# google-deepmind/dqn_zoo

Hardware: NVIDIA H100
Metric: learner_grad_steps_per_sec (higher is better)
Workload: dtype f32 (f64 sum tree)

## Files before the change

### dqn_zoo_b200/_lib.py

```python

import ctypes as C
import os

from dqn_zoo_b200 import _build

i32, i64, f32, f64, u64 = C.c_int32, C.c_int64, C.c_float, C.c_double, C.c_uint64
vp = C.c_void_p

DZ_FLAG_BAD_VALUE, DZ_FLAG_BAD_INDEX, DZ_FLAG_BAD_TARGET, DZ_FLAG_ROOT_ZERO, DZ_FLAG_NONFINITE_WEIGHT = 1, 2, 4, 8, 16
DZ_FLAG_FRAME_POOL_FULL = 32
AGENT_KINDS = {'dqn': 0, 'double_q': 1, 'prioritized': 2, 'c51': 3, 'qrdqn': 4, 'rainbow': 5, 'iqn': 6}
OPTIMIZERS = {'adam': 0, 'rmsprop': 1}


class ReplayView(C.Structure):
  _fields_ = [('d_obs', vp), ('d_action', vp), ('d_reward', vp), ('d_discount', vp), ('capacity', i64),
              ('obs_bytes', i64), ('obs_stride', i64), ('d_tree', vp), ('first_leaf', i64), ('d_live', vp),
              ('d_id_at', vp), ('d_ids', vp), ('d_flags', vp),
              ('d_frames', vp), ('frame_bytes', i64), ('frame_stride', i64), ('obs_channels', i64),
              ('frame_capacity', i64), ('d_planes', vp), ('d_refcount', vp), ('d_hashes', vp), ('d_table', vp),
              ('table_size', i64), ('d_free', vp), ('d_pool_counters', vp), ('d_add_staging', vp)]


class AddRecord(C.Structure):
# ... 82 lines not shown
    'dz_replay_gather': (i32, [C.POINTER(ReplayView), vp, i32, vp, vp, vp, vp, vp, vp]),
    'dz_replay_update_priorities': (i32, [C.POINTER(ReplayView), vp, vp, i32, f64, i64, vp]),
    'dz_learner_plan_query': (i32, [C.POINTER(LearnerConfig), C.POINTER(LearnerPlan)]),
    'dz_learner_tensor_info': (i32, [C.POINTER(LearnerConfig), i32, C.c_char_p, C.POINTER(i64), C.POINTER(i32),
                                     C.POINTER(i64)]),
    'dz_learner_create': (i32, [C.POINTER(LearnerConfig), C.POINTER(LearnerBuffers), C.POINTER(vp)]),
    'dz_learner_destroy': (None, [vp]),
    'dz_learner_update': (i32, [vp, C.POINTER(Batch), C.POINTER(UpdateOutputs), i32, vp]),
    'dz_learner_learn': (i32, [vp, C.POINTER(ReplayView), i32, C.POINTER(LearnIO), vp]),
    'dz_learner_generate_randomness': (i32, [vp, u64, vp, vp, vp]),
    'dz_learner_generate_randomness_async': (i32, [vp, u64, vp, vp, vp]),
    'dz_learner_q_values': (i32, [vp, vp, vp, vp, vp, vp]),
    'dz_learner_act_batch': (i32, [vp, vp, i32, vp, vp, vp, f32, vp, vp, vp]),
    'dz_learner_act_batch_stream_noise': (i32, [vp, vp, i32, vp, vp, f32, vp, vp, vp]),
    'dz_learner_noise_stride': (i32, [C.POINTER(LearnerConfig), C.POINTER(i64)]),
    'dz_learner_generate_stream_noise': (i32, [vp, u64, i32, vp, vp]),
    'dz_learner_sync_target': (i32, [vp, vp]),
    'dz_test_u8_to_unit': (i32, [vp, vp]),
    'dz_atari_preprocess': (i32, [vp, vp, i32, vp, vp, vp, vp, i32, vp, i32, vp]),
    'dz_atari_preprocess_band_rows': (i32, []),
    'dz_jax_uniform': (i32, [vp, vp, i32, vp, vp]),
    'dz_test_threefry2x32': (i32, [C.c_uint32, C.c_uint32, C.c_uint32, C.c_uint32, vp]),
    'dz_test_learner_buffer': (i32, [vp, C.c_char_p, vp, vp]),
    'dz_test_copy': (i32, [vp, vp, i64, vp]),
    'dz_test_learner_trace': (i32, [vp, C.c_char_p, vp]),
    'dz_test_learner_mma_path': (i32, [vp, C.c_char_p, C.POINTER(i32)]),
    'dz_debug_timeline': (i32, [vp]),
    'dz_test_tc_pgemm_work': (i64, [i32, i32, i32]),
    'dz_test_tc_pgemm': (i32, [vp, i32, i32, i32, vp, i32, i32, i32, i32, i32, vp, vp, i64, i64, i32, i64, vp, i32, vp]),
    'dz_test_umma_gemm': (i32, [vp, i32, vp, i32, i32, i32, i32, i32, vp, i32, i32, vp, i32, vp, vp, vp, vp]),
    'dz_test_umma_gemm_path': (i32, [vp, i32, vp, i32, i32, i32, i32, i32, vp, i32, i32, vp, i32, vp, vp, vp, i32, vp]),
    'dz_test_fc_forward': (i32, [i32, i32, i32, i32, i32, i32, vp, vp, vp, vp, vp, i64, vp, vp, vp, i32, vp, C.POINTER(i32),
                                 C.POINTER(i64), vp]),
    'dz_test_conv1_forward': (i32, [i32, i32, i32, i32, vp, vp, vp, i64, vp, i32, vp, vp, vp]),
}

EXPORTS = tuple(_SIGNATURES)


def library_path():
  return _build.LIB_PATH


def _load():
  path = library_path()
  if not os.path.exists(path):
    raise ImportError('dqn_zoo_b200: %s is missing — run `python -c "import __graft_entry__ as g; g.build()"` '
                      '(there is no CPU fallback)' % path)
  lib = C.CDLL(path)
  for name, (res, args) in _SIGNATURES.items():
    fn = getattr(lib, name)
    fn.restype, fn.argtypes = res, args
  return lib


lib = _load()


def check(status):
  if status != 0:
    raise _ERRORS.get(status, DzError)(lib.dz_last_error().decode())


def call(name, *args):
  check(getattr(lib, name)(*args))
```

### dqn_zoo_b200/csrc/dz_learner.cu

```cuda
#include <algorithm>
#include <cmath>
#include <map>
#include <vector>

#include "dz_async.cuh"
#include "dz_gemm.cuh"
#include "dz_tc.cuh"
#include "dz_internal.cuh"
#include "dz_umma_net.cuh"

namespace dz {


struct TensorInfo {
  std::string name;
  int64_t shape[4];
  int ndim;
  int64_t offset, count;
};

struct Dims {
  int H, W, C;
  int h1, w1, h2, w2, h3, w3;
  int feat;
// ... 1085 lines not shown
  dz_learner_config cfg;
  dz_learner_buffers buf;
  Layout lay;
  ParamOffsets po;
  Dims d;
  int B;
  int n_head[3];
  float *act1[3], *act2[3], *act3[3];
  float *h1[3][2], *out[3], *outv[3];
  float *cosf[3], *hi[3], *E0;
  float* nn_partial;
  float* conv_partial;
  float* nt_partial;
  float *dout, *doutv, *dh1[2], *dact3, *dtmp[2], *dcol, *dact2, *dact1, *dhi;
  float* tn_partial[4];
  float *loss_terms, *scalars;
  unsigned int* ticket;
  const uint8_t** rows_sample[2];
  uint8_t* recon = nullptr;
  int64_t recon_bytes = 0;
  const uint8_t** rows_act;
  int32_t* s_a; float *s_r, *s_d, *s_w;
  float* q_scratch;
  int fc_splits, head_splits, conv_splits, nt_splits;
  bool pk_on;
  struct PkImg { float* hi; float* lo; int rows_pad, red_pad; };
  PkImg pk_act[3], pk_wT[2], pk_w, pk_actT, pk_dh1T, pk_dh1, pk_cos[3], pk_weT[2], pk_dET, pk_cosT;
  bool pk_embed_bwd;
  int pk_embed_wgrad_splits;
  float *pk_fwd_partial, *pk_wgrad_partial;
  int pk_fwd_splits, pk_wgrad_splits;
  SideStream side;
  SideStream side2;
  float* norm_parts;
  UmNet* um;
  char* um_ws;
  int um_npass;
  bool opt_smem_set = false;
};

namespace {

constexpr int kNormBlocks = kNumSMs * 4;

int pick_splits(int64_t tiles, int nkb, int max_splits) {
  int best = 1;
  int64_t best_cost = -1;
  for (int s = 1; s <= max_splits; ++s) {
    int64_t cost = ceil_div(tiles * s, kNumSMs) * (ceil_div(nkb, s) + 6);
    if (best_cost < 0 || cost < best_cost) { best_cost = cost; best = s; }
  }
  return best;
}

UmNetDesc make_um_desc(const dz_learner* l);

int64_t carve(dz_learner* l, char* base) {
  const dz_learner_config& c = l->cfg;
  const Dims& d = l->d;
  const int B = c.batch;
  Bump w{base};
  const bool rb = c.kind == DZ_RAINBOW, iqn = c.kind == DZ_IQN;
  int nh[3] = {1, 1, 1};
  if (iqn) { nh[0] = c.tau_samples_s_tm1; nh[1] = c.tau_samples_policy; nh[2] = c.tau_samples_s_t; }
  for (int p = 0; p < 3; ++p) l->n_head[p] = nh[p];
  for (int p = 0; p < 3; ++p) {
// ... 551 lines not shown
  f.nsrc = nsrc; f.splits = probs[0].splits; f.stride = probs[0].split_stride; f.M = probs[0].M; f.K = probs[0].K;
  f.dual = dual ? 1 : 0; f.mask = mask; f.out = out; f.out_hi = out_hi; f.out_lo = out_lo;
  for (int q = 0; q < nsrc; ++q) { f.partial[q] = probs[q].C; f.a_scale[q] = probs[q].a_scale; }
  return f;
}
int finish_nt_batch(const FinishNT* jobs, int njobs, void* stream) {
  FinishNTBatch fb;
  memset(&fb, 0, sizeof(fb));
  long long total = 0;
  for (int j = 0; j < njobs; ++j) { fb.f[j] = jobs[j]; total = std::max(total, (long long)jobs[j].M * jobs[j].K); }
  dim3 grid((unsigned)std::min<long long>(ceil_div(total, 256), kNumSMs * 8), (unsigned)njobs);
  DZ_LAUNCH(finish_nt_kernel, grid, 256, 0, stream, fb);
  return DZ_OK;
}
int finish_nt(const GemmProblem* probs, int nsrc, const float* mask, float* out, bool dual, void* stream) {
  FinishNT f = make_finish_nt(probs, nsrc, mask, out, dual);
  return finish_nt_batch(&f, 1, stream);
}

bool split_norm_active(const dz_learner* l);

int backward_torso(dz_learner* l, const uint8_t* const* rows0, void* stream) {
  const Dims& d = l->d;
  const ParamOffsets& o = l->po;
  const int B = l->B;
  float* G = l->buf.d_grads;
  const float* P = l->buf.d_online;
  FinishTNBatch fb;
  fb.n = 0;
  GemmBatch gb;
  if (l->um && l->cfg.kind == DZ_IQN) DZ_TRY(um_split_dact3(l->um, stream));
  float* norm_parts = split_norm_active(l) ? l->norm_parts : nullptr;
  if (l->um) {
    void* ws = l->side.fork(stream, stream);
    DZ_TRY(um_wgrad_conv3(l->um, ws));
    DZ_TRY(um_wgrad_finish_layer(l->um, 3, G + o.conv_w[2], G + o.conv_b[2], norm_parts, ws));
  } else {
    GemmProblem p = zero_problem();
    set_conv(p, A_CONV_F32, l->act2[0], B, d.h2, d.w2, 64, 3, 3, 1);
    p.B = l->dact3; p.N = 64; p.ldb = 64; p.ldc = 64;
    p.Cb = G + o.conv_b[2];
    int splits = (int)std::min<int64_t>(32, ceil_div(p.M, 64));
    p.splits = splits; p.split_stride = (long long)(p.K + 1) * 64; p.C = l->tn_partial[2];
    gb.n = 1; gb.p[0] = p;
    DZ_TRY(run_tn("conv3_wgrad", gb, l->side.fork(stream, stream)));
    fb.f[fb.n++] = FinishTN{p.C, splits, p.split_stride, p.K, 64, G + o.conv_w[2], nullptr, p.Cb, nullptr, nullptr, nullptr};
  }
  if (l->um) {
    DZ_TRY(um_backward_conv3(l->um, stream));
  } else {
    GemmProblem p = zero_problem();
    p.A = l->dact3; p.lda = 64; p.M = B * d.h3 * d.w3; p.N = 64; p.K = 576;
    p.B = P + o.conv_w[2]; p.ldb = 64; p.C = l->dcol; p.ldc = 576;
    gb.n = 1; gb.p[0] = p;
    DZ_TRY(run_nt("conv3_dgrad", gb, false, stream));
    long long total = (long long)B * d.h2 * d.w2 * 64;
    DZ_LAUNCH(col2im_kernel, (unsigned)ceil_div(total, 256), 256, 0, stream, l->dcol, l->act2[0], l->dact2, B, d.h2, d.w2, 64, 3, 3, 1,
              d.h3, d.w3);
  }
  if (l->um) {
    void* ws = l->side2.fork(stream, stream);
    DZ_TRY(um_wgrad_conv2(l->um, ws));
    DZ_TRY(um_wgrad_finish_layer(l->um, 2, G + o.conv_w[1], G + o.conv_b[1], norm_parts, ws));
  } else {
    GemmProblem p = zero_problem();
    set_conv(p, A_CONV_F32, l->act1[0], B, d.h1, d.w1, 32, 4, 4, 2);
    p.B = l->dact2; p.N = 64; p.ldb = 64; p.ldc = 64;
    p.Cb = G + o.conv_b[1];
    int splits = (int)std::min<int64_t>(32, ceil_div(p.M, 64));
    p.splits = splits; p.split_stride = (long long)(p.K + 1) * 64; p.C = l->tn_partial[1];
    gb.n = 1; gb.p[0] = p;
    DZ_TRY(run_tn("conv2_wgrad", gb, l->side.fork(stream, stream)));
    fb.f[fb.n++] = FinishTN{p.C, splits, p.split_stride, p.K, 64, G + o.conv_w[1], nullptr, p.Cb, nullptr, nullptr, nullptr};
  }
  if (l->um) {
    DZ_TRY(um_backward_conv2(l->um, stream));
  } else {
    GemmProblem p = zero_problem();
    p.A = l->dact2; p.lda = 64; p.M = B * d.h2 * d.w2; p.N = 64; p.K = 512;
    p.B = P + o.conv_w[1]; p.ldb = 64; p.C = l->dcol; p.ldc = 512;
    gb.n = 1; gb.p[0] = p;
    DZ_TRY(run_nt("conv2_dgrad", gb, false, stream));
    long long total = (long long)B * d.h1 * d.w1 * 32;
    DZ_LAUNCH(col2im_kernel, (unsigned)ceil_div(total, 256), 256, 0, stream, l->dcol, l->act1[0], l->dact1, B, d.h1, d.w1, 32, 4, 4, 2,
              d.h2, d.w2);
  }
  if (l->um) {
    void* ws = l->side.fork(stream, stream);
    DZ_TRY(um_wgrad_conv1(l->um, rows0, ws));
    DZ_TRY(um_wgrad_finish_layer(l->um, 1, G + o.conv_w[0], G + o.conv_b[0], norm_parts, ws));
    DZ_TRY(l->side2.join(stream));
    return l->side.join(stream);
  } else {
    GemmProblem p = zero_problem();
    set_conv(p, A_CONV_U8, rows0, B, d.H, d.W, d.C, 8, 8, 4);
    p.B = l->dact1; p.N = 32; p.ldb = 32; p.ldc = 32;
    p.Cb = G + o.conv_b[0];
    int splits = (int)std::min<int64_t>(64, ceil_div(p.M, 64));
    p.splits = splits; p.split_stride = (long long)(p.K + 1) * 32; p.C = l->tn_partial[0];
    gb.n = 1; gb.p[0] = p;
    DZ_TRY(run_tn("conv1_wgrad", gb, l->side.fork(stream, stream)));
    fb.f[fb.n++] = FinishTN{p.C, splits, p.split_stride, p.K, 32, G + o.conv_w[0], nullptr, p.Cb, nullptr, nullptr, nullptr};
  }
  void* ws = l->side.tail(stream);
  dim3 grid((unsigned)ceil_div(577 * 64, 256), fb.n);
  DZ_LAUNCH(finish_tn_kernel, grid, 256, 0, ws, fb);
  return l->side.join(stream);
}

int backward_plain(dz_learner* l, void* stream) {
  const Dims& d = l->d;
  const ParamOffsets& o = l->po;
  const int B = l->B;
  float* G = l->buf.d_grads;
  const float* P = l->buf.d_online;
  const bool shared = l->cfg.kind == DZ_DOUBLE_Q || l->cfg.kind == DZ_PRIORITIZED;
  GemmBatch gb;
  gb.n = 1;
  {
    GemmProblem p = zero_problem();
    p.a_mode = A_PLAIN; p.A = l->h1[0][0]; p.lda = 512; p.M = B; p.K = 512;
    p.B = l->dout; p.N = d.out; p.ldb = d.out; p.ldc = d.out;
    p.C = G + o.w2[0]; p.Cb = shared ? l->scalars + 8 + kNormBlocks : G + o.b2[0];
// ... 322 lines not shown
    DZ_TRY(forward_heads_plain(l, passes, np, B, stream, um));
  }

  LossArgs L;
  memset(&L, 0, sizeof(L));
  L.kind = c.kind; L.B = B; L.A = c.num_actions; L.atoms = c.num_atoms;
  L.out0 = l->out[0]; L.out1 = l->out[1]; L.out2 = l->out[2];
  L.adv0 = l->out[0]; L.val0 = l->outv[0]; L.adv1 = l->out[1]; L.val1 = l->outv[1]; L.adv2 = l->out[2]; L.val2 = l->outv[2];
  L.a = batch->d_a_tm1; L.r = batch->d_r_t; L.disc = batch->d_discount_t; L.w = batch->d_weights; L.taus0 = batch->d_taus;
  L.vmax = c.vmax; L.bound = c.grad_error_bound; L.kappa = c.huber_param;
  L.dout = l->dout; L.dadv = l->dout; L.dval = l->doutv;
  L.per_example = out->d_per_example; L.loss_terms = l->loss_terms;
  L.priorities = (c.kind == DZ_RAINBOW || c.kind == DZ_PRIORITIZED) ? out->d_priorities : nullptr;
  if (c.kind == DZ_DQN || c.kind == DZ_DOUBLE_Q || c.kind == DZ_PRIORITIZED) {
    DZ_LAUNCH(loss_q_kernel, B, 64, 0, stream, L);
  } else if (c.kind == DZ_C51 || c.kind == DZ_RAINBOW) {
    DZ_LAUNCH_NAMED("loss_categorical_kernel", loss_categorical_staged_kernel, B, 128, categorical_loss_smem(c), stream, L);
  } else {
    if (c.kind == DZ_QRDQN) { L.N = c.num_quantiles; L.Ksel = c.num_quantiles; L.Nt = c.num_quantiles; }
    else { L.N = c.tau_samples_s_tm1; L.Ksel = c.tau_samples_policy; L.Nt = c.tau_samples_s_t; }
    size_t smem = (32 + c.num_actions + L.Nt + 2 * L.N) * sizeof(float);
    DZ_LAUNCH(loss_quantile_kernel, B, 256, smem, stream, L);
  }
  {
    void* ls = l->side.fork(stream, stream);
    DZ_LAUNCH(loss_mean_kernel, 1, 32, 0, ls, l->loss_terms, B, out->d_loss, max_seen, L.priorities);
    if (wb) DZ_TRY(launch_update_priorities(wb->view, wb->indices, wb->priorities, B, wb->alpha, wb->view->capacity, ls));
  }

  if (c.kind == DZ_RAINBOW) DZ_TRY(backward_rainbow(l, batch->d_noise, stream));
  else if (c.kind == DZ_IQN) DZ_TRY(backward_iqn(l, stream));
  else DZ_TRY(backward_plain(l, stream));
  if (split_norm_active(l)) {
    DZ_TRY(norm_fc_range(l, apply_update != 0, l->side2.fork(l->side.tail(stream), stream)));
  }
  DZ_TRY(backward_torso(l, batch->d_s_tm1_rows, stream));

  DZ_TRY(l->side2.join(stream));
  DZ_TRY(l->side.join(stream));
  DZ_TRY(run_optimizer(l, out->d_grad_norm, apply_update != 0, stream));
  return DZ_OK;
}

}


extern "C" {

int dz_learner_plan_query(const dz_learner_config* cfg, dz_learner_plan* out) {
  DZ_TRY(validate(*cfg));
  dz_learner tmp;
  tmp.um = nullptr;
  memset(&tmp.buf, 0, sizeof(tmp.buf));
  tmp.cfg = *cfg;
  tmp.lay = make_layout(*cfg);
  DZ_TRY(param_offsets(*cfg, tmp.lay, &tmp.po));
  tmp.d = make_dims(*cfg);
  tmp.B = cfg->batch;
  out->param_count = tmp.lay.total;
  out->num_tensors = (int32_t)tmp.lay.t.size();
  out->opt_state_floats = 2 * tmp.lay.total;
  out->workspace_bytes = carve(&tmp, nullptr);
  out->noise_floats = cfg->kind == DZ_RAINBOW ? 3 * noise_layout(*cfg, tmp.d).stride : 0;
  out->tau_floats = cfg->kind == DZ_IQN
                        ? (int64_t)cfg->batch * (cfg->tau_samples_s_tm1 + cfg->tau_samples_policy + cfg->tau_samples_s_t)
                        : 0;
  return DZ_OK;
// ... 13 lines not shown

int dz_learner_create(const dz_learner_config* cfg, const dz_learner_buffers* buf, dz_learner** out) {
  DZ_TRY(validate(*cfg));
  if (!buf->d_online || !buf->d_target || !buf->d_grads || !buf->d_opt_state || !buf->d_workspace || !buf->d_counters)
    return fail(DZ_EINVAL, "all learner buffers are required");
  dz_learner* l = new dz_learner();
  l->cfg = *cfg;
  l->buf = *buf;
  l->lay = make_layout(*cfg);
  l->d = make_dims(*cfg);
  l->B = cfg->batch;
  l->um = nullptr;
  int rc = param_offsets(*cfg, l->lay, &l->po);
  if (rc != DZ_OK) { delete l; return rc; }
  carve(l, static_cast<char*>(buf->d_workspace));
  if (l->um_ws) {
    UmNetDesc ud = make_um_desc(l);
    rc = um_net_create(ud, l->um_ws, &l->um);
    if (rc != DZ_OK) { delete l; return rc; }
    l->um_npass = ud.npass;
    const int um_set[3] = {0, ud.npass == 3 ? 1 : 2, 2};
    for (int i = 0; i < ud.npass; ++i) {
      const int set = um_set[i];
      l->act1[set] = um_act_f32(l->um, 1, i); l->act2[set] = um_act_f32(l->um, 2, i); l->act3[set] = um_act_f32(l->um, 3, i);
      if (ud.use_fc)
        for (int s = 0; s < ud.nstream; ++s) l->h1[set][s] = um_h1_f32(l->um, i, s);
    }
    if (ud.use_fc)
      for (int s = 0; s < ud.nstream; ++s) l->dh1[s] = um_dh1_f32(l->um, s);
    l->dact3 = um_dact_f32(l->um, 3); l->dact2 = um_dact_f32(l->um, 2); l->dact1 = um_dact_f32(l->um, 1);
  }
  cudaError_t se = l->side.create();
  if (se == cudaSuccess) se = l->side2.create();
  if (se != cudaSuccess) { dz_learner_destroy(l); return fail(DZ_ECUDA, "side streams: %s", cudaGetErrorString(se)); }
  const size_t loss_smem = categorical_loss_smem(*cfg);
  if ((cfg->kind == DZ_C51 || cfg->kind == DZ_RAINBOW) && loss_smem > 48 * 1024) {
    se = cudaFuncSetAttribute(loss_categorical_staged_kernel, cudaFuncAttributeMaxDynamicSharedMemorySize, (int)loss_smem);
    if (se != cudaSuccess) { dz_learner_destroy(l); return fail(DZ_ECUDA, "kernel attributes: %s", cudaGetErrorString(se)); }
  }
  if (l->pk_on) {
    for (int p = 0; p < 3; ++p) {
      cudaMemset(l->pk_act[p].hi, 0, pk_image_floats(l->pk_act[p].rows_pad, l->pk_act[p].red_pad) * sizeof(float));
      cudaMemset(l->pk_act[p].lo, 0, pk_image_floats(l->pk_act[p].rows_pad, l->pk_act[p].red_pad) * sizeof(float));
    }
    cudaMemset(l->pk_actT.hi, 0, pk_image_floats(l->pk_actT.rows_pad, l->pk_actT.red_pad) * sizeof(float));
    cudaMemset(l->pk_actT.lo, 0, pk_image_floats(l->pk_actT.rows_pad, l->pk_actT.red_pad) * sizeof(float));
    if (l->pk_embed_bwd) {
      cudaMemset(l->pk_dET.hi, 0, pk_image_floats(l->pk_dET.rows_pad, l->pk_dET.red_pad) * sizeof(float));
      cudaMemset(l->pk_dET.lo, 0, pk_image_floats(l->pk_dET.rows_pad, l->pk_dET.red_pad) * sizeof(float));
    }
    int rc = pk_set_ones_row(l->pk_actT.hi, l->pk_actT.rows_pad, l->d.feat, l->B * l->n_head[0], nullptr);
    if (rc != DZ_OK || cudaDeviceSynchronize() != cudaSuccess) { delete l; return rc != DZ_OK ? rc : fail(DZ_ECUDA, "packed image init"); }
  }
  cudaError_t e = cudaMemset(l->ticket, 0, 16);
  if (e != cudaSuccess) { delete l; return fail(DZ_ECUDA, "cudaMemset: %s", cudaGetErrorString(e)); }
  *out = l;
  return DZ_OK;
}

void dz_learner_destroy(dz_learner* l) {
  if (!l) return;
  um_net_destroy(l->um);
  l->side.destroy();
  l->side2.destroy();
  if (l->recon) cudaFree(l->recon);
  delete l;
}

int dz_learner_update(dz_learner* l, const dz_batch* batch, const dz_update_outputs* out, int32_t apply_update, void* stream) {
  return update_impl(l, batch, out, apply_update, nullptr, nullptr, stream);
}

int dz_learner_learn(dz_learner* l, const dz_replay_view* replay, int32_t prioritized, const dz_learn_io* io, void* stream) {
  const int B = l->B;
  BatchExtras ex{l->rows_sample[0], l->rows_sample[1], l->s_a, l->s_r, l->s_d, prioritized ? l->s_w : nullptr, 1};
  if (replay->obs_bytes != (int64_t)l->d.H * l->d.W * l->d.C) return fail(DZ_EINVAL, "replay observation size does not match the network");
  if (replay->d_planes) {
    const int64_t need = (int64_t)B * 2 * replay->obs_stride;
    if (need > l->recon_bytes) {
      cudaStreamCaptureStatus cs = cudaStreamCaptureStatusNone;
      DZ_CUDA_OK(cudaStreamIsCapturing((cudaStream_t)stream, &cs));
      if (cs != cudaStreamCaptureStatusNone)
        return fail(DZ_EINVAL, "the first dz_learner_learn on a frame-deduplicated replay must run eagerly, not in a capture");
      if (l->recon) DZ_CUDA_OK(cudaFree(l->recon));
      l->recon = nullptr;
      l->recon_bytes = 0;
      DZ_CUDA_OK(cudaMalloc(&l->recon, need));
      l->recon_bytes = need;
    }
    ex.recon = l->recon;
  }
  const bool pack_aside = l->um != nullptr;
  if (pack_aside) {
    void* ws = l->side.fork(stream, stream);
    DZ_TRY(um_pack_weights(l->um, ws));
  }
  DZ_TRY(launch_sample(replay, prioritized, &io->sample_in, &io->sample_out, B, ex, stream));
// ... 189 lines not shown
```

### dqn_zoo_b200/csrc/dz_umma.cu

```cuda
#include <cudaTypedefs.h>

#include "dz_umma_host.cuh"

namespace dz {

namespace {

PFN_cuTensorMapEncodeTiled_v12000 encode_fn() {
  static PFN_cuTensorMapEncodeTiled_v12000 fn = nullptr;
  if (!fn) {
    void* p = nullptr;
    cudaDriverEntryPointQueryResult q;
    if (cudaGetDriverEntryPoint("cuTensorMapEncodeTiled", &p, cudaEnableDefault, &q) == cudaSuccess && q == cudaDriverEntryPointSuccess)
      fn = reinterpret_cast<PFN_cuTensorMapEncodeTiled_v12000>(p);
  }
  return fn;
}

}

int UmPlan::add_map(const void* base, int rank, const uint64_t* dims, const uint64_t* strides_bytes, const uint32_t* box) {
  auto fn = encode_fn();
  if (!fn) { fail(DZ_ECUDA, "cuTensorMapEncodeTiled entry point not available"); return -1; }
  cuuint64_t gd[5] = {1, 1, 1, 1, 1};
// ... 74 lines not shown
      ops[oi].map = (uint32_t)slot;
    }
  }
  return DZ_OK;
}

void UmPlan::release() {
  if (d_maps) cudaFree(d_maps);
  if (d_probs) cudaFree(d_probs);
  if (d_ctas) cudaFree(d_ctas);
  if (d_ops) cudaFree(d_ops);
  d_maps = nullptr; d_probs = nullptr; d_ctas = nullptr; d_ops = nullptr;
}

int UmPlan::upload() {
  release();
  if (maps.empty() || probs.empty() || ctas.empty() || ops.empty()) return fail(DZ_EINVAL, "empty umma plan");
  DZ_CUDA_OK(cudaMalloc(&d_maps, maps.size() * sizeof(CUtensorMap)));
  DZ_CUDA_OK(cudaMalloc(&d_probs, probs.size() * sizeof(UmProblem)));
  DZ_CUDA_OK(cudaMalloc(&d_ctas, ctas.size() * sizeof(UmCta)));
  DZ_CUDA_OK(cudaMalloc(&d_ops, ops.size() * sizeof(UmTmaOp)));
  DZ_CUDA_OK(cudaMemcpy(d_maps, maps.data(), maps.size() * sizeof(CUtensorMap), cudaMemcpyHostToDevice));
  DZ_CUDA_OK(cudaMemcpy(d_probs, probs.data(), probs.size() * sizeof(UmProblem), cudaMemcpyHostToDevice));
  DZ_CUDA_OK(cudaMemcpy(d_ctas, ctas.data(), ctas.size() * sizeof(UmCta), cudaMemcpyHostToDevice));
  DZ_CUDA_OK(cudaMemcpy(d_ops, ops.data(), ops.size() * sizeof(UmTmaOp), cudaMemcpyHostToDevice));
  return DZ_OK;
}

int UmPlan::configure() {
  static bool done = false;
  if (done) return DZ_OK;
  DZ_CUDA_OK(cudaFuncSetAttribute(um::umma_gemm_kernel<32>, cudaFuncAttributeMaxDynamicSharedMemorySize, 227 * 1024));
  DZ_CUDA_OK(cudaFuncSetAttribute(um::umma_gemm_kernel<64>, cudaFuncAttributeMaxDynamicSharedMemorySize, 227 * 1024));
  DZ_CUDA_OK(cudaFuncSetAttribute(um::umma_fc_kernel<32>, cudaFuncAttributeMaxDynamicSharedMemorySize, 227 * 1024));
  DZ_CUDA_OK(cudaFuncSetAttribute(um::umma_fc_kernel<64>, cudaFuncAttributeMaxDynamicSharedMemorySize, 227 * 1024));
  DZ_CUDA_OK(cudaFuncSetAttribute(um::wgmma_gemm_kernel<32>, cudaFuncAttributeMaxDynamicSharedMemorySize, 227 * 1024));
  DZ_CUDA_OK(cudaFuncSetAttribute(um::wgmma_gemm_kernel<64>, cudaFuncAttributeMaxDynamicSharedMemorySize, 227 * 1024));
  done = true;
  return DZ_OK;
}

bool UmPlan::wgmma_eligible(const UmLaunch& l) const {
  for (int ci = l.cta0; ci < l.cta0 + l.nctas; ++ci) {
    const UmProblem& pr = probs[ctas[ci].prob];
    for (const UmOperand* o : {&pr.A, &pr.B})
      if (o->mn_major || o->nparts != 2 || o->convert) return false;
    if (pr.ksteps != 4) return false;
  }
  return true;
}

bool UmPlan::fc_eligible(const UmLaunch& l) const {
  for (int ci = l.cta0; ci < l.cta0 + l.nctas; ++ci) {
    const UmCta& c = ctas[ci];
    const int np = c.nprob > 1 ? (int)c.nprob : 1;
    if (np > um::kFcMaxProbs) return false;
    for (int q = 0; q < np; ++q) {
      const UmProblem& pr = probs[c.prob + q];
      if (!pr.A.mn_major || pr.A.lbo != 4096u || pr.A.part_bytes * (uint32_t)np != 16384u) return false;
      if (pr.A.convert != 2 && !(pr.A.convert == 1 && pr.A.scale_r == nullptr)) return false;
      if (pr.B.mn_major || pr.B.nparts != 2 || pr.B.convert) return false;
      if (pr.ksteps != 4 || pr.red_per_stage != 32 || pr.epi != UM_EPI_PARTIAL || pr.sc_i != 1) return false;
      if (q > 0 && (pr.A.part_bytes != probs[c.prob].A.part_bytes || pr.A.convert != probs[c.prob].A.convert ||
                    pr.B.part_bytes != probs[c.prob].B.part_bytes))
        return false;
    }
    if (2 * 16384u / (uint32_t)np + (uint32_t)np * 2u * probs[c.prob].B.part_bytes > l.stage_bytes) return false;
  }
  return true;
}

int UmPlan::launch(const char* tag, const UmLaunch& l, void* stream, long long* d_trace, int path) const {
  if (l.nctas <= 0) return DZ_OK;
  if (!d_ctas) return fail(DZ_EINVAL, "umma plan not uploaded");
  if (l.stages < 1 || l.stages > um::kStagesMax || l.stage_bytes % 1024) return fail(DZ_EINVAL, "umma launch geometry");
  for (int ci = l.cta0; ci < l.cta0 + l.nctas; ++ci) {
    const UmProblem& pr = probs[ctas[ci].prob];
    const uint32_t want = pr.B.mn_major ? (uint32_t)(l.njt / 32) * pr.B.lbo : (uint32_t)l.njt * 128u;
    if (pr.A.nparts != 2 || pr.B.nparts != 2 || pr.B.part_bytes != want)
      return fail(DZ_EINVAL, "umma launch: operands must be hi/lo pairs and the B tile must span NJT rows");
  }
  const int stages = l.stages;
  const size_t smem = um_smem_bytes(stages, l.stage_bytes);
  if (smem > 227 * 1024) return fail(DZ_EINVAL, "umma launch needs too much shared memory");
  if ((size_t)stages * l.stage_bytes < (size_t)128 * l.njt * 4) return fail(DZ_EINVAL, "umma launch: stage buffers smaller than the store-phase staging tile");
  const int v = l.njt == 32 ? 0 : 1;
  if (l.njt != 32 && l.njt != 64) return fail(DZ_EINVAL, "umma launch: NJT must be 32 or 64");
  if (path != UM_PATH_AUTO && path != UM_PATH_MMA_SYNC && path != UM_PATH_WGMMA && path != UM_PATH_CONVERTERS)
    return fail(DZ_EINVAL, "umma launch: unknown MMA path");
  const bool wg = path == UM_PATH_AUTO ? wgmma_eligible(l) : path == UM_PATH_WGMMA;
  if (wg && !wgmma_eligible(l)) return fail(DZ_EINVAL, "umma launch: the wgmma path needs K-major, pre-split operands and four k-steps per stage");
  if (wg)
    for (int ci = l.cta0; ci < l.cta0 + l.nctas; ++ci)
      if (um_wgmma_min_stage(probs[ctas[ci].prob].A.part_bytes) > l.stage_bytes) return fail(DZ_EINVAL, "umma launch: stage too small for the wgmma A reads");
  DZ_TRY(configure());
  um::UmMaps lm;
  for (int q = 0; q < l.nmaps; ++q) lm.m[q] = maps[l.map_ids[q]];
  for (int q = l.nmaps; q < um::kMaxMapsPerLaunch; ++q) lm.m[q] = maps[l.map_ids[0]];
  if (wg) {
    if (v == 0)
      DZ_LAUNCH_NAMED(tag, um::wgmma_gemm_kernel<32>, (unsigned)l.nctas, um::kThreadsW, smem, stream, lm, d_ctas + l.cta0, d_probs, d_ops, l.nmaps,
                      stages, l.stage_bytes, d_trace);
    else
      DZ_LAUNCH_NAMED(tag, um::wgmma_gemm_kernel<64>, (unsigned)l.nctas, um::kThreadsW, smem, stream, lm, d_ctas + l.cta0, d_probs, d_ops, l.nmaps,
                      stages, l.stage_bytes, d_trace);
    return DZ_OK;
  }
  if (path != UM_PATH_CONVERTERS && fc_eligible(l)) {
    if (v == 0)
      DZ_LAUNCH_NAMED(tag, um::umma_fc_kernel<32>, (unsigned)l.nctas, um::kThreadsF, smem, stream, lm, d_ctas + l.cta0, d_probs, d_ops, l.nmaps,
                      stages, l.stage_bytes, d_trace);
    else
      DZ_LAUNCH_NAMED(tag, um::umma_fc_kernel<64>, (unsigned)l.nctas, um::kThreadsF, smem, stream, lm, d_ctas + l.cta0, d_probs, d_ops, l.nmaps,
                      stages, l.stage_bytes, d_trace);
    return DZ_OK;
  }
  for (int ci = l.cta0; ci < l.cta0 + l.nctas; ++ci)
    if (ctas[ci].nprob > 1) return fail(DZ_EINVAL, "umma launch: CTAs that serve several problems need umma_fc_kernel");
  if (v == 0)
    DZ_LAUNCH_NAMED(tag, um::umma_gemm_kernel<32>, (unsigned)l.nctas, um::kThreadsU, smem, stream, lm, d_ctas + l.cta0, d_probs, d_ops, l.nmaps, stages,
                    l.stage_bytes, d_trace);
  else
    DZ_LAUNCH_NAMED(tag, um::umma_gemm_kernel<64>, (unsigned)l.nctas, um::kThreadsU, smem, stream, lm, d_ctas + l.cta0, d_probs, d_ops, l.nmaps, stages,
                    l.stage_bytes, d_trace);
  return DZ_OK;
}

namespace {
__global__ void um_split_kernel(const float* __restrict__ x, float* __restrict__ hi, float* __restrict__ lo, long long n) {
  dz::pdl_enter();
  long long i = blockIdx.x * (long long)blockDim.x + threadIdx.x;
  if (i < n) {
    float h, l;
    tc::split_tf32(x[i], h, l);
    hi[i] = h;
    lo[i] = l;
  }
}
}

int um_split(const float* x, float* hi, float* lo, long long n, void* stream) {
  DZ_LAUNCH(um_split_kernel, (unsigned)ceil_div(n, 256), 256, 0, stream, x, hi, lo, n);
  return DZ_OK;
}

}

// ... 90 lines not shown
```

### dqn_zoo_b200/csrc/dz_umma.cuh

```cuda
#pragma once
#include <cuda.h>

#include "dz_async.cuh"
#include "dz_internal.cuh"
#include "dz_tc.cuh"

namespace dz {

struct UmTmaOp {
  uint32_t map;
  uint32_t smem_off;
  int32_t c[5];
  uint32_t pad;
};

struct UmOperand {
  uint32_t part_bytes;
  uint32_t nparts;
  uint32_t convert;
  uint32_t mn_major;
  uint32_t lbo;
  const float* scale_r;
  const float* scale_i;
};
// ... 345 lines not shown
  if (!direct && warp >= 2 && warp < 14) {
    if (warp >= 6 && !any_conv) dz::pdl_enter();
    bar_sync_coop();
    if (warp < 6) {
      const int m0 = (warp - 2) * 32;
#pragma unroll
      for (int mt = 0; mt < 2; ++mt)
#pragma unroll
        for (int nt = 0; nt < NT; ++nt)
#pragma unroll
          for (int e = 0; e < 4; e += 2) {
            const int r = m0 + frag_row(mt, e), c = frag_col(nt, e);
            *reinterpret_cast<float2*>(reinterpret_cast<float*>(stage_chunk<NJT>(stage_base, r, c >> 2)) + (c & 3)) =
                make_float2(sum[mt][nt][e], sum[mt][nt][e + 1]);
          }
    }
    bar_sync_coop();
    store_tile<NJT>(p, cta, stage_base, threadIdx.x - 64);
  }
  if (tr && warp == 2 && lane == 0) trace[321] = clock64();
  if (tr && threadIdx.x == 0) trace[322] = clock64();
}

__device__ __forceinline__ void stamp_if(long long* addr, bool pred) {
  asm volatile("{\n.reg .pred p;\n.reg .b64 c;\nsetp.ne.b32 p, %1, 0;\nmov.u64 c, %%clock64;\n@p st.global.b64 [%0], c;\n}\n" ::"l"(addr),
               "r"((int)pred)
               : "memory");
}

constexpr int kFcMmaWarps = 8;
constexpr int kThreadsF = (1 + kFcMmaWarps) * 32;
constexpr int kFcMaxProbs = 2;

template <int NJT>
__global__ void __launch_bounds__(kThreadsF, 1)
    umma_fc_kernel(const __grid_constant__ UmMaps maps, const UmCta* __restrict__ ctas, const UmProblem* __restrict__ probs,
                   const UmTmaOp* __restrict__ ops, int nmaps, int stages, uint32_t stage_bytes, long long* __restrict__ trace) {
  if (threadIdx.x < nmaps) prefetch_tensormap(&maps.m[threadIdx.x]);
  extern __shared__ uint8_t smem_raw[];
  uint8_t* smem = smem_raw + smem_pad_1024(smem_raw);
  const bool tr = trace != nullptr && blockIdx.x == 0;
  const UmCta cta = ctas[blockIdx.x];
  const int ST = stages;
  const int nst = (int)cta.nstages;
  const int P = cta.nprob > 1 ? 2 : 1;

  uint64_t* full = reinterpret_cast<uint64_t*>(smem);
  uint64_t* empty = full + 2 * kStagesMax;
  UmProblem* p_smem = reinterpret_cast<UmProblem*>(smem + 1024);
  UmTmaOp* ops_smem = reinterpret_cast<UmTmaOp*>(smem + 2048);
  uint8_t* stage_base = smem + kCtlBytes;
  static_assert(kFcMaxProbs * sizeof(UmProblem) <= 1024, "problem copies do not fit their slot");

  const int warp = threadIdx.x >> 5, lane = threadIdx.x & 31;
  {
    const uint4* src = reinterpret_cast<const uint4*>(probs + cta.prob);
    uint4* dst = reinterpret_cast<uint4*>(p_smem);
    for (int i = threadIdx.x; i < P * (int)(sizeof(UmProblem) / 16); i += kThreadsF) dst[i] = src[i];
    const int nvec = min(nst * (int)cta.ops_per_stage, kMaxOpsPerCta) * 2;
    const uint4* osrc = reinterpret_cast<const uint4*>(ops + cta.op0);
    uint4* odst = reinterpret_cast<uint4*>(ops_smem);
    for (int i = threadIdx.x; i < nvec; i += kThreadsF) odst[i] = osrc[i];
  }
  if (warp == 0 && lane == 0) {
    for (int s = 0; s < ST; ++s) { mbar_init(&full[s], 1); mbar_init(&empty[s], kFcMmaWarps); }
    fence_mbarrier_init();
  }
// ... 4 lines not shown
    int s = 0;
    uint32_t ph = 0;
    uint32_t st_addr = smem_u32(stage_base);
    int oi = 0;
    dz::pdl_enter();
    if (tr && lane == 0) { trace[323] = clock64(); trace[324] = clock64(); }
    for (int it = 0; it < nst; ++it) {
      mbar_wait(&empty[s], ph ^ 1u);
      if (lane == 0) mbar_expect_tx(&full[s], cta.tx_bytes);
      __syncwarp();
      if (lane < nops) {
        const int o = oi + lane;
        const UmTmaOp op = o < kMaxOpsPerCta ? ops_smem[o] : ops[cta.op0 + o];
        tma_load_5d(st_addr + op.smem_off, &maps.m[op.map], &full[s], op.c[0], op.c[1], op.c[2], op.c[3], op.c[4]);
      }
      if (tr && lane == 0 && it < 64) trace[it] = clock64();
      __syncwarp();
      oi += nops;
      ++s; st_addr += stage_bytes;
      if (s == ST) { s = 0; ph ^= 1u; st_addr = smem_u32(stage_base); }
    }
    return;
  }

  const int w = warp - 1, wpp = kFcMmaWarps / P;
  const int q = w / wpp, m0 = 16 * (w - q * wpp);
  const bool lead = w == 0 && lane == 0;
  const UmProblem& p = p_smem[q];
  const int g = lane >> 2, t = lane & 3;
  const uint32_t a_part = p.A.part_bytes, a_lbo = p.A.lbo;
  const uint8_t* b_first = stage_base + a_part * 2 + (uint32_t)q * 2u * p.B.part_bytes;
  const uint32_t b_part = p.B.part_bytes;
  const bool noisy = p.A.convert == 2;
  const float* __restrict__ eps_in = p.A.scale_r;
  constexpr int NT = NJT / 8;
  float sum[1][NT][4];
#pragma unroll
  for (int nt = 0; nt < NT; ++nt)
#pragma unroll
    for (int e = 0; e < 4; ++e) sum[0][nt][e] = 0.f;
  auto b_off = [](int n, int k) { return sw128_kmajor(n, k); };
  dz::pdl_enter();
  float eo[2] = {1.f, 1.f};
  if (noisy) {
    eo[0] = p.A.scale_i[cta.i0 + m0 + g];
    eo[1] = p.A.scale_i[cta.i0 + m0 + g + 8];
  }
  int s = 0, r0 = cta.r0;
  uint32_t ph = 0;
  for (int it = 0; it < nst; ++it) {
    mbar_wait(&full[s], ph);
    stamp_if(trace + 64 + it, tr && lead && it < 64);
    const uint8_t* mu = stage_base + (size_t)s * stage_bytes;
    const uint8_t* sg = mu + a_part;
    const uint8_t* bh = b_first + (size_t)s * stage_bytes;
#pragma unroll(NJT == 32 ? 4 : 2)
    for (int ks = 0; ks < 4; ++ks) {
      uint32_t ah[1][4], al[1][4];
      float ei[2] = {1.f, 1.f};
      if (noisy) { ei[0] = eps_in[r0 + 8 * ks + t]; ei[1] = eps_in[r0 + 8 * ks + t + 4]; }
#pragma unroll
      for (int e = 0; e < 4; ++e) {
        const uint32_t o = sw128_mnmajor(m0 + g + (e & 1) * 8, 8 * ks + t + (e >> 1) * 4, a_lbo);
        float v = *reinterpret_cast<const float*>(mu + o);
        if (noisy) {
          const float f = ei[e >> 1] * eo[e & 1];
          v = fmaf(*reinterpret_cast<const float*>(sg + o), f, v);
        }
        float hh, ll;
        split_tf32(v, hh, ll);
        ah[0][e] = __float_as_uint(hh);
        al[0][e] = __float_as_uint(ll);
      }
      warp_mma_3xtf32<1, NT>(sum, ah, al, true, bh, bh + b_part, 0, 8 * ks, b_off);
    }
    __syncwarp();
    if (lane == 0) mbar_arrive(&empty[s]);
    stamp_if(trace + 128 + it, tr && lead && it < 64);
    r0 += 32;
    if (++s == ST) { s = 0; ph ^= 1u; }
  }
  if (lead) asm volatile("griddepcontrol.launch_dependents;" ::: "memory");
  if (tr && lead) trace[320] = clock64();
  float* dst = p.C + (long long)cta.split * p.split_stride;
  const long long sc_j = p.sc_j;
#pragma unroll
  for (int e = 0; e < 4; e += 2) {
    const int i = cta.i0 + m0 + frag_row(0, e);
    if (i >= p.MI) continue;
    const float sc = p.scale_i ? p.scale_i[i] : 1.0f;
#pragma unroll
    for (int nt = 0; nt < NT; ++nt)
#pragma unroll
      for (int h = 0; h < 2; ++h) {
        const int j = frag_col(nt, e + h);
        if (j < p.NJ) dst[i + (long long)j * sc_j] = sum[0][nt][e + h] * sc;
// ... 173 lines not shown
```

### dqn_zoo_b200/csrc/dz_umma_net.cu

```cuda
#include <algorithm>

#include "dz_umma_net.cuh"

namespace dz {

enum NetLaunch : int { kConv2Fwd, kConv3Fwd, kConv3Dgrad, kConv2Dgrad, kFcFwd, kFcDgrad, kConv3Wgrad, kConv2Wgrad, kNumNetLaunches };
struct NetLaunchName { const char* tag; const char* noisy; };
constexpr NetLaunchName kNetLaunchNames[kNumNetLaunches] = {
    {"conv2_fwd", nullptr},   {"conv3_fwd", nullptr},    {"conv3_dgrad", nullptr}, {"conv2_dgrad", nullptr},
    {"fc1_fwd", "noisy1_fwd"}, {"fc1_dgrad", "noisy1_dgrad"}, {"conv3_wgrad", nullptr}, {"conv2_wgrad", nullptr}};

constexpr int kConvN[3] = {32, 64, 64}, kConvK[3] = {256, 512, 576};
constexpr int kConvFwdFloats = kConvN[0] * kConvK[0] + kConvN[1] * kConvK[1] + kConvN[2] * kConvK[2];

struct UmNet {
  UmNetDesc d;
  int h1, w1, h2, w2, h3, w3, feat, PB;
  UmPlan plan;
  float *act_hi[3], *act_lo[3], *act_f32[3];
  float *dact_hi[3], *dact_lo[3], *dact_f32[3];
  float *h1_buf, *dh1_f32, *dh1_hi, *dh1_lo;
  float *fc_part, *fcd_part;
  int fc_splits, fcd_splits, fc_nprob, fcd_nsrc;
  float *wf_hi[2][3], *wf_lo[2][3], *wd3_hi, *wd3_lo, *wd2_hi, *wd2_lo;
// ... 1424 lines not shown
    if (noisy) { d.off_fc_sw[s] = off_sw[s]; d.noise_off_in[s] = off_in[s]; d.noise_off_out[s] = off_out[s]; }
  }
  for (int p = 0; p < 3; ++p) d.noise_apply[p] = p;
  d.noise_stride = noise_stride;
  if (!um_net_supported(d)) return fail(DZ_EINVAL, "fc forward test: geometry not supported by the tensor-core path");
  char* ws = nullptr;
  DZ_CUDA_OK(cudaMalloc(&ws, (size_t)um_net_workspace_bytes(d)));
  UmNet* n = nullptr;
  int rc = net_create(d, ws, &n, per_pass != 0);
  if (rc == DZ_OK) rc = um_split(x, n->act_hi[2], n->act_lo[2], (long long)n->PB * n->feat, stream);
  if (rc == DZ_OK && noisy) rc = apply_noise(n, noise, stream);
  if (rc == DZ_OK) rc = n->plan.launch("fc1_fwd", n->launches[kFcFwd], stream, nullptr, per_pass ? UM_PATH_CONVERTERS : UM_PATH_AUTO);
  if (rc == DZ_OK) {
    const size_t bytes = (size_t)npass * nstream * n->fc_splits * B * 512 * sizeof(float);
    if (cudaMemcpyAsync(d_part, n->fc_part, bytes, cudaMemcpyDeviceToDevice, (cudaStream_t)stream) != cudaSuccess ||
        cudaStreamSynchronize((cudaStream_t)stream) != cudaSuccess)
      rc = fail(DZ_ECUDA, "fc forward test: %s", cudaGetErrorString(cudaGetLastError()));
  }
  if (rc == DZ_OK) {
    *splits = n->fc_splits;
    int64_t wb = 0;
    const UmLaunch& l = n->launches[kFcFwd];
    for (int ci = l.cta0; ci < l.cta0 + l.nctas; ++ci) {
      const UmCta& c = n->plan.ctas[ci];
      wb += (int64_t)c.nstages * (noisy ? 2 : 1) * n->plan.probs[c.prob].A.part_bytes;
    }
    *weight_bytes = wb;
  }
  if (n) um_net_destroy(n);
  cudaFree(ws);
  return rc;
}

extern "C" int dz_test_conv1_forward(int32_t B, int32_t H, int32_t W, int32_t npass, const float* online, const float* target,
                                     const int64_t* off_conv_w, int64_t off_conv_b1, const uint8_t* const* const* rows,
                                     int32_t path, float* d_hi, float* d_lo, void* stream) {
  if (npass < 1 || npass > 3) return fail(DZ_EINVAL, "conv1 forward test: npass 1..3");
  if (path != UM_PATH_MMA_SYNC && path != UM_PATH_WGMMA) return fail(DZ_EINVAL, "conv1 forward test: path 1 (mma.sync) or 2 (wgmma)");
  UmNetDesc d;
  memset(&d, 0, sizeof(d));
  d.B = B; d.H = H; d.W = W; d.npass = npass;
  d.pass_target[0] = 0; d.pass_target[1] = npass == 3 ? 0 : 1; d.pass_target[2] = 1;
  d.online = online; d.target = target;
  for (int L = 0; L < 3; ++L) d.off_conv_w[L] = off_conv_w[L];
  d.off_conv_b[0] = off_conv_b1;
  if (!um_net_supported(d)) return fail(DZ_EINVAL, "conv1 forward test: geometry not supported by the tensor-core path");
  char* ws = nullptr;
  DZ_CUDA_OK(cudaMalloc(&ws, (size_t)um_net_workspace_bytes(d)));
  UmNet* n = nullptr;
  int rc = net_create(d, ws, &n, false);
  if (rc == DZ_OK) rc = um_pack_weights(n, stream);
  if (rc == DZ_OK) rc = launch_conv1(n, rows, stream, path == UM_PATH_MMA_SYNC);
  if (rc == DZ_OK) {
    const size_t bytes = (size_t)npass * B * n->h1 * n->w1 * 32 * sizeof(float);
    if (cudaMemcpyAsync(d_hi, n->act_hi[0], bytes, cudaMemcpyDeviceToDevice, (cudaStream_t)stream) != cudaSuccess ||
        cudaMemcpyAsync(d_lo, n->act_lo[0], bytes, cudaMemcpyDeviceToDevice, (cudaStream_t)stream) != cudaSuccess ||
        cudaStreamSynchronize((cudaStream_t)stream) != cudaSuccess)
      rc = fail(DZ_ECUDA, "conv1 forward test: %s", cudaGetErrorString(cudaGetLastError()));
  }
  if (n) um_net_destroy(n);
  cudaFree(ws);
  return rc;
}
```

### include/dqn_zoo_b200.h

```cpp
#ifndef DQN_ZOO_B200_H_
#define DQN_ZOO_B200_H_

#include <stddef.h>
#include <stdint.h>

#ifdef __cplusplus
extern "C" {
#endif

#define DZ_OK 0
#define DZ_EINVAL (-1)
#define DZ_ECUDA (-2)
#define DZ_ERANGE (-3)
#define DZ_ESTATE (-4)

const char* dz_last_error(void);
const char* dz_build_info(void);
int64_t dz_launch_count(void);
int dz_profile_begin(void);
int dz_profile_end(char* out, int64_t cap);


int dz_sumtree_rebuild(double* d_nodes, int64_t first_leaf, int64_t n_valid, void* stream);

// ... 226 lines not shown
  const int32_t* d_bounds;
  const int32_t* d_kk;
  int32_t ksize, in_size, out_size;
} dz_resample_axis;
int dz_atari_preprocess(const uint8_t* const* d_frame_a, const uint8_t* const* d_frame_b, int32_t n_env,
                        const dz_resample_axis* horizontal, const dz_resample_axis* vertical,
                        uint8_t* const* d_stacks, const int32_t* d_counts, int32_t stack, const double* luma3,
                        int32_t max_band_rows, void* stream);
int32_t dz_atari_preprocess_band_rows(void);

int dz_jax_uniform(const uint32_t* d_keys, const int64_t* counts, int32_t nblocks, float* d_out, void* stream);
int dz_test_threefry2x32(uint32_t k0, uint32_t k1, uint32_t c0, uint32_t c1, uint32_t* out2);

int dz_test_learner_buffer(dz_learner* l, const char* name, float** d_ptr, int64_t* count);
int dz_test_copy(void* d_dst, const void* d_src, int64_t bytes, void* stream);
int dz_test_learner_trace(dz_learner* l, const char* tag, long long* d_trace);
int dz_test_learner_mma_path(dz_learner* l, const char* tag, int32_t* path);
int dz_debug_timeline(unsigned long long* d_buf);
int64_t dz_test_tc_pgemm_work(int32_t a_rows, int32_t b_rows, int32_t red);
int dz_test_tc_pgemm(const float* d_A, int32_t a_rows, int32_t a_ld, int32_t a_red_contig, const float* d_B,
                     int32_t b_rows, int32_t b_ld, int32_t b_red_contig, int32_t red, int32_t a_ones_row,
                     float* d_work, float* d_C, int64_t sc_i, int64_t sc_j, int32_t splits, int64_t split_stride,
                     const float* d_bias, int32_t relu, void* stream);
int dz_test_umma_gemm(const float* d_A, int32_t a_mn_major, const float* d_B, int32_t b_mn_major, int32_t MI, int32_t NJ,
                      int32_t R, int32_t convert, const float* d_scale_r, int32_t stages, int32_t epi_rows,
                      const float* d_bias, int32_t relu, float* d_C, float* d_hi, float* d_lo, void* stream);
int dz_test_umma_gemm_path(const float* d_A, int32_t a_mn_major, const float* d_B, int32_t b_mn_major, int32_t MI, int32_t NJ,
                           int32_t R, int32_t convert, const float* d_scale_r, int32_t stages, int32_t epi_rows,
                           const float* d_bias, int32_t relu, float* d_C, float* d_hi, float* d_lo, int32_t path, void* stream);
int dz_test_fc_forward(int32_t B, int32_t H, int32_t W, int32_t npass, int32_t nstream, int32_t noisy, const float* online,
                       const float* target, const int64_t* off_w, const int64_t* off_sw, const float* noise, int64_t noise_stride,
                       const int64_t* off_in, const int64_t* off_out, const float* x, int32_t per_pass, float* d_part,
                       int32_t* splits, int64_t* weight_bytes, void* stream);
int dz_test_conv1_forward(int32_t B, int32_t H, int32_t W, int32_t npass, const float* online, const float* target,
                          const int64_t* off_conv_w, int64_t off_conv_b1, const uint8_t* const* const* rows, int32_t path,
                          float* d_hi, float* d_lo, void* stream);

#ifdef __cplusplus
}
#endif
#endif
```

Baseline: 2908.

## Route FC input-gradient through fused FC kernel and rebalance side streams

Extends the specialised umma_fc_kernel with a K-major A-operand variant so the FC input-gradient problem (single-problem, K-major) can use the fused FC path instead of the generic one. The noisy-layer input epsilons are now prefetched one stage ahead and broadcast by warp shuffles rather than re-read from global memory per k-step. Conv weight-gradient work moves to a new third side stream, and the FC norm now runs on the first side stream, changing the overlap between backward stages. A test entry point for the FC dgrad is added. The stream reshuffle risks new serialisation or ordering hazards.

After: 3061 (median of 6 runs). 1.05x the previous value.

```diff
diff --git a/dqn_zoo_b200/_lib.py b/dqn_zoo_b200/_lib.py
--- a/dqn_zoo_b200/_lib.py
+++ b/dqn_zoo_b200/_lib.py
@@ -138,6 +138,7 @@
     'dz_test_umma_gemm_path': (i32, [vp, i32, vp, i32, i32, i32, i32, i32, vp, i32, i32, vp, i32, vp, vp, vp, i32, vp]),
     'dz_test_fc_forward': (i32, [i32, i32, i32, i32, i32, i32, vp, vp, vp, vp, vp, i64, vp, vp, vp, i32, vp, C.POINTER(i32),
                                  C.POINTER(i64), vp]),
+    'dz_test_fc_dgrad': (i32, [i32, i32, i32, i32, i32, vp, vp, vp, vp, vp, vp, vp, i32, vp, C.POINTER(i32), vp]),
     'dz_test_conv1_forward': (i32, [i32, i32, i32, i32, vp, vp, vp, i64, vp, i32, vp, vp, vp]),
 }
 
diff --git a/dqn_zoo_b200/csrc/dz_learner.cu b/dqn_zoo_b200/csrc/dz_learner.cu
--- a/dqn_zoo_b200/csrc/dz_learner.cu
+++ b/dqn_zoo_b200/csrc/dz_learner.cu
@@ -1141,6 +1141,7 @@
   int pk_fwd_splits, pk_wgrad_splits;
   SideStream side;
   SideStream side2;
+  SideStream side3;
   float* norm_parts;
   UmNet* um;
   char* um_ws;
@@ -1758,7 +1759,7 @@
   if (l->um && l->cfg.kind == DZ_IQN) DZ_TRY(um_split_dact3(l->um, stream));
   float* norm_parts = split_norm_active(l) ? l->norm_parts : nullptr;
   if (l->um) {
-    void* ws = l->side.fork(stream, stream);
+    void* ws = l->side3.fork(stream, stream);
     DZ_TRY(um_wgrad_conv3(l->um, ws));
     DZ_TRY(um_wgrad_finish_layer(l->um, 3, G + o.conv_w[2], G + o.conv_b[2], norm_parts, ws));
   } else {
@@ -1812,9 +1813,10 @@
               d.h2, d.w2);
   }
   if (l->um) {
-    void* ws = l->side.fork(stream, stream);
+    void* ws = l->side3.fork(stream, stream);
     DZ_TRY(um_wgrad_conv1(l->um, rows0, ws));
     DZ_TRY(um_wgrad_finish_layer(l->um, 1, G + o.conv_w[0], G + o.conv_b[0], norm_parts, ws));
+    DZ_TRY(l->side3.join(stream));
     DZ_TRY(l->side2.join(stream));
     return l->side.join(stream);
   } else {
@@ -2203,7 +2205,7 @@
   else if (c.kind == DZ_IQN) DZ_TRY(backward_iqn(l, stream));
   else DZ_TRY(backward_plain(l, stream));
   if (split_norm_active(l)) {
-    DZ_TRY(norm_fc_range(l, apply_update != 0, l->side2.fork(l->side.tail(stream), stream)));
+    DZ_TRY(norm_fc_range(l, apply_update != 0, l->side.tail(stream)));
   }
   DZ_TRY(backward_torso(l, batch->d_s_tm1_rows, stream));
 
@@ -2283,6 +2285,7 @@
   }
   cudaError_t se = l->side.create();
   if (se == cudaSuccess) se = l->side2.create();
+  if (se == cudaSuccess) se = l->side3.create();
   if (se != cudaSuccess) { dz_learner_destroy(l); return fail(DZ_ECUDA, "side streams: %s", cudaGetErrorString(se)); }
   const size_t loss_smem = categorical_loss_smem(*cfg);
   if ((cfg->kind == DZ_C51 || cfg->kind == DZ_RAINBOW) && loss_smem > 48 * 1024) {
@@ -2314,6 +2317,7 @@
   um_net_destroy(l->um);
   l->side.destroy();
   l->side2.destroy();
+  l->side3.destroy();
   if (l->recon) cudaFree(l->recon);
   delete l;
 }
diff --git a/dqn_zoo_b200/csrc/dz_umma.cu b/dqn_zoo_b200/csrc/dz_umma.cu
--- a/dqn_zoo_b200/csrc/dz_umma.cu
+++ b/dqn_zoo_b200/csrc/dz_umma.cu
@@ -130,8 +130,10 @@
   if (done) return DZ_OK;
   DZ_CUDA_OK(cudaFuncSetAttribute(um::umma_gemm_kernel<32>, cudaFuncAttributeMaxDynamicSharedMemorySize, 227 * 1024));
   DZ_CUDA_OK(cudaFuncSetAttribute(um::umma_gemm_kernel<64>, cudaFuncAttributeMaxDynamicSharedMemorySize, 227 * 1024));
-  DZ_CUDA_OK(cudaFuncSetAttribute(um::umma_fc_kernel<32>, cudaFuncAttributeMaxDynamicSharedMemorySize, 227 * 1024));
-  DZ_CUDA_OK(cudaFuncSetAttribute(um::umma_fc_kernel<64>, cudaFuncAttributeMaxDynamicSharedMemorySize, 227 * 1024));
+  DZ_CUDA_OK(cudaFuncSetAttribute(um::umma_fc_kernel<32, false>, cudaFuncAttributeMaxDynamicSharedMemorySize, 227 * 1024));
+  DZ_CUDA_OK(cudaFuncSetAttribute(um::umma_fc_kernel<64, false>, cudaFuncAttributeMaxDynamicSharedMemorySize, 227 * 1024));
+  DZ_CUDA_OK(cudaFuncSetAttribute(um::umma_fc_kernel<32, true>, cudaFuncAttributeMaxDynamicSharedMemorySize, 227 * 1024));
+  DZ_CUDA_OK(cudaFuncSetAttribute(um::umma_fc_kernel<64, true>, cudaFuncAttributeMaxDynamicSharedMemorySize, 227 * 1024));
   DZ_CUDA_OK(cudaFuncSetAttribute(um::wgmma_gemm_kernel<32>, cudaFuncAttributeMaxDynamicSharedMemorySize, 227 * 1024));
   DZ_CUDA_OK(cudaFuncSetAttribute(um::wgmma_gemm_kernel<64>, cudaFuncAttributeMaxDynamicSharedMemorySize, 227 * 1024));
   done = true;
@@ -155,7 +157,9 @@
     if (np > um::kFcMaxProbs) return false;
     for (int q = 0; q < np; ++q) {
       const UmProblem& pr = probs[c.prob + q];
-      if (!pr.A.mn_major || pr.A.lbo != 4096u || pr.A.part_bytes * (uint32_t)np != 16384u) return false;
+      if (pr.A.mn_major != probs[ctas[l.cta0].prob].A.mn_major) return false;
+      if (pr.A.mn_major ? pr.A.lbo != 4096u : np != 1) return false;
+      if (pr.A.part_bytes * (uint32_t)np != 16384u) return false;
       if (pr.A.convert != 2 && !(pr.A.convert == 1 && pr.A.scale_r == nullptr)) return false;
       if (pr.B.mn_major || pr.B.nparts != 2 || pr.B.convert) return false;
       if (pr.ksteps != 4 || pr.red_per_stage != 32 || pr.epi != UM_EPI_PARTIAL || pr.sc_i != 1) return false;
@@ -205,12 +209,11 @@
     return DZ_OK;
   }
   if (path != UM_PATH_CONVERTERS && fc_eligible(l)) {
-    if (v == 0)
-      DZ_LAUNCH_NAMED(tag, um::umma_fc_kernel<32>, (unsigned)l.nctas, um::kThreadsF, smem, stream, lm, d_ctas + l.cta0, d_probs, d_ops, l.nmaps,
-                      stages, l.stage_bytes, d_trace);
-    else
-      DZ_LAUNCH_NAMED(tag, um::umma_fc_kernel<64>, (unsigned)l.nctas, um::kThreadsF, smem, stream, lm, d_ctas + l.cta0, d_probs, d_ops, l.nmaps,
-                      stages, l.stage_bytes, d_trace);
+    const bool ak = !probs[ctas[l.cta0].prob].A.mn_major;
+    auto kern = v == 0 ? (ak ? um::umma_fc_kernel<32, true> : um::umma_fc_kernel<32, false>)
+                       : (ak ? um::umma_fc_kernel<64, true> : um::umma_fc_kernel<64, false>);
+    DZ_LAUNCH_NAMED(tag, kern, (unsigned)l.nctas, um::kThreadsF, smem, stream, lm, d_ctas + l.cta0, d_probs, d_ops, l.nmaps, stages,
+                    l.stage_bytes, d_trace);
     return DZ_OK;
   }
   for (int ci = l.cta0; ci < l.cta0 + l.nctas; ++ci)
diff --git a/dqn_zoo_b200/csrc/dz_umma.cuh b/dqn_zoo_b200/csrc/dz_umma.cuh
--- a/dqn_zoo_b200/csrc/dz_umma.cuh
+++ b/dqn_zoo_b200/csrc/dz_umma.cuh
@@ -401,7 +401,7 @@
 constexpr int kThreadsF = (1 + kFcMmaWarps) * 32;
 constexpr int kFcMaxProbs = 2;
 
-template <int NJT>
+template <int NJT, bool AK>
 __global__ void __launch_bounds__(kThreadsF, 1)
     umma_fc_kernel(const __grid_constant__ UmMaps maps, const UmCta* __restrict__ ctas, const UmProblem* __restrict__ probs,
                    const UmTmaOp* __restrict__ ops, int nmaps, int stages, uint32_t stage_bytes, long long* __restrict__ trace) {
@@ -472,7 +472,7 @@
   const uint8_t* b_first = stage_base + a_part * 2 + (uint32_t)q * 2u * p.B.part_bytes;
   const uint32_t b_part = p.B.part_bytes;
   const bool noisy = p.A.convert == 2;
-  const float* __restrict__ eps_in = p.A.scale_r;
+  const float* __restrict__ eps_r = p.A.scale_r;
   constexpr int NT = NJT / 8;
   float sum[1][NT][4];
 #pragma unroll
@@ -483,12 +483,15 @@
   dz::pdl_enter();
   float eo[2] = {1.f, 1.f};
   if (noisy) {
-    eo[0] = p.A.scale_i[cta.i0 + m0 + g];
-    eo[1] = p.A.scale_i[cta.i0 + m0 + g + 8];
-  }
+    eo[0] = p.A.scale_i[min(cta.i0 + m0 + g, p.MI - 1)];
+    eo[1] = p.A.scale_i[min(cta.i0 + m0 + g + 8, p.MI - 1)];
+  }
+  float er_next = noisy ? eps_r[cta.r0 + lane] : 1.f;
   int s = 0, r0 = cta.r0;
   uint32_t ph = 0;
   for (int it = 0; it < nst; ++it) {
+    const float er = er_next;
+    if (noisy && it + 1 < nst) er_next = eps_r[r0 + 32 + lane];
     mbar_wait(&full[s], ph);
     stamp_if(trace + 64 + it, tr && lead && it < 64);
     const uint8_t* mu = stage_base + (size_t)s * stage_bytes;
@@ -497,11 +500,11 @@
 #pragma unroll(NJT == 32 ? 4 : 2)
     for (int ks = 0; ks < 4; ++ks) {
       uint32_t ah[1][4], al[1][4];
-      float ei[2] = {1.f, 1.f};
-      if (noisy) { ei[0] = eps_in[r0 + 8 * ks + t]; ei[1] = eps_in[r0 + 8 * ks + t + 4]; }
+      const float ei[2] = {__shfl_sync(0xffffffffu, er, 8 * ks + t), __shfl_sync(0xffffffffu, er, 8 * ks + t + 4)};
 #pragma unroll
       for (int e = 0; e < 4; ++e) {
-        const uint32_t o = sw128_mnmajor(m0 + g + (e & 1) * 8, 8 * ks + t + (e >> 1) * 4, a_lbo);
+        const int m = m0 + g + (e & 1) * 8, k = 8 * ks + t + (e >> 1) * 4;
+        const uint32_t o = AK ? sw128_kmajor(m, k) : sw128_mnmajor(m, k, a_lbo);
         float v = *reinterpret_cast<const float*>(mu + o);
         if (noisy) {
           const float f = ei[e >> 1] * eo[e & 1];
diff --git a/dqn_zoo_b200/csrc/dz_umma_net.cu b/dqn_zoo_b200/csrc/dz_umma_net.cu
--- a/dqn_zoo_b200/csrc/dz_umma_net.cu
+++ b/dqn_zoo_b200/csrc/dz_umma_net.cu
@@ -1480,6 +1480,39 @@
   return rc;
 }
 
+extern "C" int dz_test_fc_dgrad(int32_t B, int32_t H, int32_t W, int32_t nstream, int32_t noisy, const float* online, const int64_t* off_w,
+                                const int64_t* off_sw, const float* noise, const int64_t* off_in, const int64_t* off_out, const float* g,
+                                int32_t converters, float* d_part, int32_t* splits, void* stream) {
+  if (nstream < 1 || nstream > 2) return fail(DZ_EINVAL, "fc input-gradient test: nstream 1..2");
+  UmNetDesc d;
+  memset(&d, 0, sizeof(d));
+  d.B = B; d.H = H; d.W = W; d.npass = 1;
+  d.online = online; d.target = online;
+  d.use_fc = 1; d.nstream = nstream; d.noisy = noisy ? 1 : 0;
+  for (int s = 0; s < nstream; ++s) {
+    d.off_fc_w[s] = off_w[s];
+    if (noisy) { d.off_fc_sw[s] = off_sw[s]; d.noise_off_in[s] = off_in[s]; d.noise_off_out[s] = off_out[s]; }
+  }
+  if (!um_net_supported(d)) return fail(DZ_EINVAL, "fc input-gradient test: geometry not supported by the tensor-core path");
+  char* ws = nullptr;
+  DZ_CUDA_OK(cudaMalloc(&ws, (size_t)um_net_workspace_bytes(d)));
+  UmNet* n = nullptr;
+  int rc = net_create(d, ws, &n, false);
+  if (rc == DZ_OK) rc = um_split(g, n->dh1_hi, n->dh1_lo, (long long)nstream * B * 512, stream);
+  if (rc == DZ_OK && noisy) rc = apply_noise(n, noise, stream);
+  if (rc == DZ_OK) rc = n->plan.launch("fc1_dgrad", n->launches[kFcDgrad], stream, nullptr, converters ? UM_PATH_CONVERTERS : UM_PATH_AUTO);
+  if (rc == DZ_OK) {
+    const size_t bytes = (size_t)nstream * n->fcd_splits * B * n->feat * sizeof(float);
+    if (cudaMemcpyAsync(d_part, n->fcd_part, bytes, cudaMemcpyDeviceToDevice, (cudaStream_t)stream) != cudaSuccess ||
+        cudaStreamSynchronize((cudaStream_t)stream) != cudaSuccess)
+      rc = fail(DZ_ECUDA, "fc input-gradient test: %s", cudaGetErrorString(cudaGetLastError()));
+  }
+  if (rc == DZ_OK) *splits = n->fcd_splits;
+  if (n) um_net_destroy(n);
+  cudaFree(ws);
+  return rc;
+}
+
 extern "C" int dz_test_conv1_forward(int32_t B, int32_t H, int32_t W, int32_t npass, const float* online, const float* target,
                                      const int64_t* off_conv_w, int64_t off_conv_b1, const uint8_t* const* const* rows,
                                      int32_t path, float* d_hi, float* d_lo, void* stream) {
diff --git a/include/dqn_zoo_b200.h b/include/dqn_zoo_b200.h
--- a/include/dqn_zoo_b200.h
+++ b/include/dqn_zoo_b200.h
@@ -282,6 +282,9 @@
                        const float* target, const int64_t* off_w, const int64_t* off_sw, const float* noise, int64_t noise_stride,
                        const int64_t* off_in, const int64_t* off_out, const float* x, int32_t per_pass, float* d_part,
                        int32_t* splits, int64_t* weight_bytes, void* stream);
+int dz_test_fc_dgrad(int32_t B, int32_t H, int32_t W, int32_t nstream, int32_t noisy, const float* online, const int64_t* off_w,
+                     const int64_t* off_sw, const float* noise, const int64_t* off_in, const int64_t* off_out, const float* g,
+                     int32_t converters, float* d_part, int32_t* splits, void* stream);
 int dz_test_conv1_forward(int32_t B, int32_t H, int32_t W, int32_t npass, const float* online, const float* target,
                           const int64_t* off_conv_w, int64_t off_conv_b1, const uint8_t* const* const* rows, int32_t path,
                           float* d_hi, float* d_lo, void* stream);
```
